# tiddoloos/Scaling-RGCN-training

Hardware: AMD Instinct MI355X
Metric: edges/s per RGCN layer (fwd+bwd) (higher is better)
Workload: dtype f32 (contraction: bf16x3 split of fp32 operands, fp32 accumulate)

## Files before the change

scaling_rgcn_training_amd/csrc/rgcn_dw_tile.hip:

```cpp
#include "rgcn_kernels_shared.h"

namespace rgcn {

constexpr int kDwTileT = 320;
constexpr int kDwTileWalkers = 64;
constexpr int kDwTileMaxRel = 32;
constexpr int kDwFlushUnits = 128;

struct DwTileArgs {
    const int* rel_order;
    const int* chunk_cnt;
    const int* chunk_tile;
    const int* slot_src;
    const float* slot_w;
    const int* slot_row;
    const int* slot_src2;
    const int* walk_ptr;
    const float* x;
    const float* g;
    unsigned x_bytes, g_bytes;
    float* slabs;
    int ldx, ldg, dout4, n_tiles, n_owned, num_rel, walkers;
};

template <bool SPLIT, bool PAIRS = false>
__global__ void __launch_bounds__(512, 2) rgcn_dw_tile_kernel(const DwTileArgs a) {
    constexpr int T = kDwTileT, NP = 64, HS = 8;
    extern __shared__ __attribute__((aligned(16))) float lds[];
    const int tid = threadIdx.x;
    const int lane = tid & 63;
    const int wave = __builtin_amdgcn_readfirstlane(tid >> 6);
    const int quarter = (blockIdx.x >> 3) & 3, p = (blockIdx.x & 7) | ((blockIdx.x >> 5) << 3);
    const int rel = 8 * quarter + wave;
    const bool have = rel < a.num_rel;
    const int t0 = (int)((long)p * a.n_tiles / a.walkers), t1 = (int)((long)(p + 1) * a.n_tiles / a.walkers);
    if (t1 <= t0) return;
    const int i0 = have ? ldc(a.walk_ptr, (long)rel * (a.walkers + 1) + p) : 0;
    const int nun = have ? ldc(a.walk_ptr, (long)rel * (a.walkers + 1) + p + 1) - i0 : 0;
    const int ml = lane & 15, kq = lane >> 4;
    const __amdgpu_buffer_rsrc_t rx = make_rsrc(a.x, a.x_bytes), rg = make_rsrc(a.g, a.g_bytes);
    const unsigned colb = 16u * (unsigned)ml;
    const unsigned rbx = (unsigned)a.ldx * 4u, rbg = (unsigned)a.ldg * 4u;
    const unsigned gcol = ml < a.dout4 ? colb : 0xFFFFFFF0u;
    const unsigned grow = ml < a.dout4 ? rbg : 0u;
    const int perm = kq * 4;
// ... 5 lines not shown
        for (int jb = 0; jb < 4; ++jb) acc[ia][jb] = (f32x4){0.f, 0.f, 0.f, 0.f};

    auto dma_tile = [&](int t, int b) {
        float* base = lds + b * T * NP;
        for (int i = wave; i < T / 4; i += 8) {
            const unsigned row = (unsigned)(t * T + 4 * i + kq);
            dma16_buf(rg, __umul24(row, grow) + gcol, base + i * 4 * NP);
        }
    };
    struct Idx {
        int h, g;
        float w;
        int h2;
    };
    auto unit_of = [&](int k) { return ldc(a.rel_order, i0 + (k < nun ? k : (nun > 0 ? nun - 1 : 0))); };
    auto load_idx = [&](int unit) {
        const size_t base = (size_t)unit * kChunk + lane;
        int h2 = 0;
        if constexpr (PAIRS) h2 = a.slot_src2[(size_t)unit * 8 + (lane & 7)];
        return Idx{a.slot_src[base], a.slot_row[base], a.slot_w[base], h2};
    };
    auto issue_half = [&](f32x4 (&a4)[HS], f32x4& pair, const Idx& ix, int h) {
        if constexpr (PAIRS) {
            const int i2 = __builtin_amdgcn_ds_bpermute(perm + 16 * h, ix.h2);
            pair = __builtin_bit_cast(f32x4, __builtin_amdgcn_raw_buffer_load_b128(rx, (int)(__umul24((unsigned)i2, rbx) + colb), 0, 0));
        }
        int ih[HS];
#pragma unroll
        for (int s = 0; s < HS; ++s) ih[s] = __builtin_amdgcn_ds_bpermute(perm + 16 * (HS * h + s), ix.h);
#pragma unroll
        for (int s = 0; s < HS; ++s)
            a4[s] = __builtin_bit_cast(f32x4, __builtin_amdgcn_raw_buffer_load_b128(rx, (int)(__umul24((unsigned)ih[s], rbx) + colb), 0, 0));
    };
    auto compute_half = [&](f32x4 (&a4)[HS], const f32x4& pair, const Idx& ix, int h, int ngrp, int nks, const float* gbuf, int tile_row0) {
        if constexpr (PAIRS) a4[0] += pair;
        const unsigned loc = (unsigned)(ix.g - tile_row0);
        const int goff = (int)((loc < (unsigned)T ? loc : (unsigned)(T - 1)) * (unsigned)(NP * 4));
        float wv[HS];
        f32x4 g4[HS];
#pragma unroll
        for (int s = 0; s < HS; ++s) {
            wv[s] = __builtin_bit_cast(float, __builtin_amdgcn_ds_bpermute(perm + 16 * (HS * h + s), __builtin_bit_cast(int, ix.w)));
            const int o = __builtin_amdgcn_ds_bpermute(perm + 16 * (HS * h + s), goff);
            g4[s] = *(const f32x4*)((const char*)gbuf + o + colb);
        }
#pragma unroll
        for (int gi = 0; gi < 2; ++gi) {
            if (2 * h + gi < ngrp) {
#pragma unroll
                for (int t = 0; t < 4; ++t) {
                    const int s = 4 * gi + t;
                    f32x4 bv = g4[s] * wv[s];
                    asm volatile("s_nop 4" : "+v"(bv));
#pragma unroll
                    for (int ia = 0; ia < 4; ++ia)
#pragma unroll
                        for (int jb = 0; jb < 4; ++jb)
                            asm volatile("v_mfma_f32_16x16x4_f32 %0, %1, %2, %0" : "+v"(acc[ia][jb]) : "v"(a4[s][ia]), "v"(bv[jb]));
                }
            }
        }
    };

    auto compute_half3 = [&](f32x4 (&a4)[HS], const f32x4& pair, const Idx& ix, int h, int ngrp, const float* gbuf, int tile_row0) {
        if (2 * h >= ngrp) return;
        if constexpr (PAIRS) a4[0] += pair;
        const unsigned loc = (unsigned)(ix.g - tile_row0);
        const int goff = (int)((loc < (unsigned)T ? loc : (unsigned)(T - 1)) * (unsigned)(NP * 4));
        float wv[HS];
        f32x4 g4[HS];
#pragma unroll
        for (int s = 0; s < HS; ++s) {
            wv[s] = __builtin_bit_cast(float, __builtin_amdgcn_ds_bpermute(perm + 16 * (HS * h + s), __builtin_bit_cast(int, ix.w)));
            const int o = __builtin_amdgcn_ds_bpermute(perm + 16 * (HS * h + s), goff);
            g4[s] = *(const f32x4*)((const char*)gbuf + o + colb);
        }
        u32x4 ap[3][4];
#pragma unroll
        for (int ia = 0; ia < 4; ++ia) {
            float v0[4], v1[4];
            unsigned pc[4];
#pragma unroll
            for (int jp = 0; jp < 4; ++jp) { v0[jp] = a4[2 * jp][ia]; v1[jp] = a4[2 * jp + 1][ia]; }
#pragma unroll
            for (int piece = 0; piece < 3; ++piece) {
#pragma unroll
                for (int jp = 0; jp < 4; ++jp) pc[jp] = cvt_pk_bf16(v0[jp], v1[jp]);
                __builtin_amdgcn_sched_barrier(0);
#pragma unroll
                for (int jp = 0; jp < 4; ++jp) ap[piece][ia][jp] = pc[jp];
                if (piece < 2) {
#pragma unroll
                    for (int jp = 0; jp < 4; ++jp) {
                        v0[jp] -= __uint_as_float(pc[jp] << 16);
                        v1[jp] -= __uint_as_float(pc[jp] & 0xFFFF0000u);
                    }
                    __builtin_amdgcn_sched_barrier(0);
                }
            }
        }
        constexpr int pa[6] = {2, 1, 1, 0, 0, 0}, pb[6] = {0, 1, 0, 2, 1, 0};
        auto cut_b = [&](int jb, u32x4 (&bp)[3]) {
#pragma unroll
            for (int jp = 0; jp < 4; ++jp) {
                unsigned h_, m_, l_;
                split3_pair(g4[2 * jp][jb] * wv[2 * jp], g4[2 * jp + 1][jb] * wv[2 * jp + 1], h_, m_, l_);
                bp[0][jp] = h_; bp[1][jp] = m_; bp[2][jp] = l_;
            }
        };
// ... 38 lines not shown
                    __builtin_amdgcn_sched_group_barrier(0x002, 3, 0);
                }
            }
            __builtin_amdgcn_sched_barrier(0);
        }
        __builtin_amdgcn_s_setprio(0);
    };

    auto pin_loads = [] { asm volatile("" ::: "memory"); };
    float* const slab = a.slabs + ((size_t)p * a.num_rel + (have ? rel : 0)) * (64 * 64);
    auto fold_into_slab = [&](float sgn) {
        if (!have) return;
        if constexpr (!SPLIT) asm volatile("s_nop 15\n\ts_nop 15" ::: "memory");
#pragma unroll
        for (int ia = 0; ia < 4; ++ia)
#pragma unroll
            for (int r = 0; r < 4; ++r) {
                f32x4* q = (f32x4*)(slab + (4 * (4 * kq + r) + ia) * NP + 4 * ml);
                f32x4 v = *q;
#pragma unroll
                for (int jb = 0; jb < 4; ++jb) {
                    v[jb] += sgn * acc[ia][jb][r];
                    acc[ia][jb][r] = 0.f;
                }
                *q = v;
            }
    };
    float sgn = 1.f;
    const int fold_period = min(SPLIT ? kDwFlushUnits : 4 * kDwFlushUnits, max(16, nun >> 3));
    int fold_left = fold_period;
    dma_tile(t0, 0);
    int k = 0;
    int uid_cur = unit_of(0), uid_nxt = unit_of(1), uid_nn = unit_of(2);
    int cnt_cur = ldc(a.chunk_cnt, uid_cur), tile_cur = nun > 0 ? ldc(a.chunk_tile, uid_cur) : t1;
    int cnt_nxt = ldc(a.chunk_cnt, uid_nxt), tile_nxt = nun > 1 ? ldc(a.chunk_tile, uid_nxt) : t1;
    Idx ix_cur = load_idx(uid_cur), ix_nxt = load_idx(uid_nxt);
    f32x4 s0[HS], s1[HS];
    f32x4 p0 = {0.f, 0.f, 0.f, 0.f}, p1 = {0.f, 0.f, 0.f, 0.f};
    if (nun > 0) issue_half(s0, p0, ix_cur, 0);
    constexpr int kInFlight = 11 + (PAIRS ? 2 : 0);
    bool walked = nun > 0;
    for (int t = t0; t < t1; ++t) {
        if (walked) asm volatile("s_waitcnt vmcnt(%0)" ::"n"(kInFlight) : "memory");
        else asm volatile("s_waitcnt vmcnt(0)" ::: "memory");
        wg_barrier();
        const int b = (t - t0) & 1;
        if (t + 1 < t1) dma_tile(t + 1, b ^ 1);
        walked = false;
        const float* gbuf = lds + b * T * NP;
        while (k < nun && tile_cur == t) {
            const int ngrp = (cnt_cur + 15) >> 4, nks = (cnt_cur + 3) >> 2;
            walked = true;
            issue_half(s1, p1, ix_cur, 1);
            pin_loads();
            __builtin_amdgcn_sched_barrier(0);
            if constexpr (SPLIT) ix_cur.w *= sgn;
            if constexpr (SPLIT) compute_half3(s0, p0, ix_cur, 0, ngrp, gbuf, t * T);
            else compute_half(s0, p0, ix_cur, 0, ngrp, nks, gbuf, t * T);
            __builtin_amdgcn_sched_barrier(0);
            const Idx ix_nn = load_idx(uid_nn);
            issue_half(s0, p0, ix_nxt, 0);
            pin_loads();
            __builtin_amdgcn_sched_barrier(0);
            if constexpr (SPLIT) compute_half3(s1, p1, ix_cur, 1, ngrp, gbuf, t * T);
            else compute_half(s1, p1, ix_cur, 1, ngrp, nks, gbuf, t * T);
            __builtin_amdgcn_sched_barrier(0);
            ++k;
            if (--fold_left == 0) {
                fold_left = fold_period;
                fold_into_slab(sgn);
                if (SPLIT) sgn = -sgn;
            }
            ix_cur = ix_nxt;
            ix_nxt = ix_nn;
            uid_cur = uid_nxt;
            uid_nxt = uid_nn;
            uid_nn = unit_of(k + 2);
            cnt_cur = cnt_nxt;
            tile_cur = k < nun ? tile_nxt : t1;
            cnt_nxt = ldc(a.chunk_cnt, uid_nxt);
            tile_nxt = k + 1 < nun ? ldc(a.chunk_tile, uid_nxt) : t1;
        }
    }
    asm volatile("s_waitcnt vmcnt(0)" ::: "memory");
    asm volatile("s_nop 15\n\ts_nop 15" ::: "memory");
    fold_into_slab(sgn);
}

__global__ void rgcn_dw_walk_table_kernel(const int* __restrict__ rel_order, const int* __restrict__ chunk_rel,
                                          const int* __restrict__ chunk_tile, int n_units, int n_tiles, int num_rel, int walkers,
                                          int* __restrict__ walk_ptr) {
    const int i = blockIdx.x * blockDim.x + threadIdx.x;
    if (i >= num_rel * (walkers + 1)) return;
    const int r = i / (walkers + 1), p = i - r * (walkers + 1);
    const long target = (long)r * n_tiles + (long)p * n_tiles / walkers;
    int lo = 0, hi = n_units;
    while (lo < hi) {
        const int mid = (lo + hi) >> 1;
        const int c = rel_order[mid];
        if ((long)chunk_rel[c] * n_tiles + chunk_tile[c] < target) lo = mid + 1; else hi = mid;
    }
    walk_ptr[i] = lo;
}

__global__ void rgcn_dw_tile_reduce_kernel(const float* __restrict__ slabs, int walkers, int num_rel, int din, int dout,
                                           float* __restrict__ d_weight) {
    const int r = blockIdx.x;
    for (int e = blockIdx.y * blockDim.x + threadIdx.x; e < din * dout; e += gridDim.y * blockDim.x) {
        const int kk = e / dout, n = e - kk * dout;
        float sum = 0.f;
        for (int w = 0; w < walkers; ++w) sum += slabs[((size_t)w * num_rel + r) * (64 * 64) + kk * 64 + n];
        d_weight[(size_t)r * din * dout + e] = sum;
    }
}


// ... 11 lines not shown

extern "C" int rgcn_dw_tiles_walk(const rgcn_plan_t* plan, int32_t* walk_ptr, void* stream) {
    int st;
    if ((st = check_device()) != RGCN_OK) return st;
    if ((st = check_plan(plan)) != RGCN_OK) return st;
    if (walk_ptr == nullptr) return RGCN_ERR_NULL;
    if (plan->tile != kDwTileT || plan->chunk != 64 || (plan->layout != 0 && plan->layout != 5) || plan->num_relations > kDwTileMaxRel) return RGCN_ERR_PLAN;
    const int n = plan->num_relations * (kDwTileWalkers + 1);
    hipLaunchKernelGGL(rgcn_dw_walk_table_kernel, dim3((n + 255) / 256), dim3(256), 0, (hipStream_t)stream, plan->rel_order,
                       plan->chunk_rel, plan->chunk_tile, plan->n_units, plan->n_tiles, plan->num_relations, kDwTileWalkers, walk_ptr);
    return (int)hipGetLastError();
}

extern "C" size_t rgcn_bwd_dw_tiles_workspace_bytes(int num_relations) {
    return num_relations > 0 ? sizeof(float) * (size_t)kDwTileWalkers * num_relations * 64 * 64 : 0;
}

extern "C" int rgcn_bwd_dw_tiles(const rgcn_plan_t* plan, const int32_t* walk_ptr, const float* x, int ldx, int din, const float* g,
                                 int ldg, int dout, void* workspace, size_t workspace_bytes, float* d_weight, unsigned flags,
                                 void* stream) {
    int st = check_plan(plan);
    if (st != RGCN_OK) return st;
    if (!walk_ptr || !x || !g || !workspace || !d_weight) return RGCN_ERR_NULL;
    if ((st = check_stride(ldx, din)) != RGCN_OK) return st;
    if ((st = check_stride(ldg, dout)) != RGCN_OK) return st;
    if (padded_width(din) != 64 || padded_width(dout) != 64) return RGCN_ERR_WIDTH;
    if (plan->tile != kDwTileT || plan->chunk != 64 || (plan->layout != 0 && plan->layout != 5) || plan->num_relations > kDwTileMaxRel) return RGCN_ERR_PLAN;
    if (workspace_bytes < rgcn_bwd_dw_tiles_workspace_bytes(plan->num_relations)) return RGCN_ERR_WORKSPACE;
    if ((st = check_device()) != RGCN_OK) return st;
    DwTileArgs a;
    a.rel_order = plan->rel_order;
    a.chunk_cnt = plan->chunk_cnt;
    a.chunk_tile = plan->chunk_tile;
    a.slot_src = plan->slot_src;
    a.slot_w = plan->slot_w;
    a.slot_row = plan->slot_row;
    a.walk_ptr = walk_ptr;
    a.x = x;
    a.g = g;
    a.x_bytes = buffer_bytes(plan->n_nodes, ldx, flags);
    a.g_bytes = buffer_bytes(plan->n_owned, ldg, flags);
    if (a.x_bytes == 0 || a.g_bytes == 0) return RGCN_ERR_ADDRESS;
    a.slabs = (float*)workspace;
    a.ldx = ldx;
    a.ldg = ldg;
    a.dout4 = (dout + 3) / 4;
    a.n_tiles = plan->n_tiles;
    a.n_owned = plan->n_owned;
    a.num_rel = plan->num_relations;
    a.walkers = kDwTileWalkers;
    hipStream_t s = (hipStream_t)stream;
    const size_t lds = sizeof(float) * 2 * kDwTileT * 64;
    const bool split = (flags & RGCN_FLAG_SPLIT_PRODUCERS) != 0;
    a.slot_src2 = plan->layout == 5 ? plan->slot_src2 : nullptr;
    if (plan->layout == 5 && a.slot_src2 == nullptr) return RGCN_ERR_NULL;
    hipError_t e = split ? allow_full_lds<rgcn_dw_tile_kernel<true>>() : allow_full_lds<rgcn_dw_tile_kernel<false>>();
    if (e != hipSuccess) return (int)e;
    e = hipMemsetAsync(workspace, 0, rgcn_bwd_dw_tiles_workspace_bytes(plan->num_relations), s);
    if (e != hipSuccess) return (int)e;
    if (a.slot_src2 != nullptr) {
        e = split ? allow_full_lds<rgcn_dw_tile_kernel<true, true>>() : allow_full_lds<rgcn_dw_tile_kernel<false, true>>();
        if (e != hipSuccess) return (int)e;
        if (split) hipLaunchKernelGGL((rgcn_dw_tile_kernel<true, true>), dim3(4 * kDwTileWalkers), dim3(512), lds, s, a);
        else hipLaunchKernelGGL((rgcn_dw_tile_kernel<false, true>), dim3(4 * kDwTileWalkers), dim3(512), lds, s, a);
    } else if (split) hipLaunchKernelGGL(rgcn_dw_tile_kernel<true>, dim3(4 * kDwTileWalkers), dim3(512), lds, s, a);
    else hipLaunchKernelGGL(rgcn_dw_tile_kernel<false>, dim3(4 * kDwTileWalkers), dim3(512), lds, s, a);
// ... 5 lines not shown
```

scaling_rgcn_training_amd/csrc/rgcn_plan.hip:

```cpp
#include <hip/hip_runtime.h>
#include <stdint.h>
#include <string.h>
#include "../../include/rgcn_mi355x.h"

namespace rgcn_planner {

typedef unsigned long long u64;
typedef unsigned int u32;

constexpr int kSortItems = 32;
constexpr int kSegKeys = 64 * kSortItems;
constexpr int kSortThreads = 256;
constexpr int kScanThreads = 256;
constexpr int kScanItems = 8;
constexpr int kScanBlock = kScanThreads * kScanItems;

__host__ __device__ inline int bits_for(u64 max_value) {
    int b = 1;
    while ((max_value >> b) != 0 && b < 64) ++b;
    return b;
}

__device__ inline u32 block_exclusive_scan(u32 v, u32* lds_wave_tot, u32& block_total) {
    const int lane = threadIdx.x & 63, wave = threadIdx.x >> 6;
// ... 582 lines not shown
        while (j + len < n && lrow[j + len] == lrow[j] && lw[j + len] == lw[j]) ++len;
        u32 k = 0;
        while (k < len) {
            const bool as_pair = k + 1 < len && pair_left > 0;
            u32 u, sl;
            if (as_pair) {
                u = next_pair[0] < pairs_in[0] ? 0u : 1u;
                const u32 kk = next_pair[u]++;
                sl = kk < 4u ? kk : 28u + kk;
                --pair_left;
            } else {
                u = single_u;
                for (;;) {
                    while (next_single[u] < unit_heads(u) && is_pair_place(u, next_single[u])) ++next_single[u];
                    if (next_single[u] < unit_heads(u)) break;
                    single_u = ++u;
                }
                sl = next_single[u]++;
            }
            const size_t g = base + (size_t)u * 64u + sl;
            slot_src[g] = lsrc[j + k];
            slot_w[g] = __uint_as_float(lw[j + k]);
            slot_row[g] = lrow[j + k];
            if (as_pair) {
                slot_src2[(size_t)(c + u) * 8u + (sl < 4u ? sl : sl - 28u)] = lsrc[j + k + 1];
                k += 2;
            } else {
                k += 1;
            }
        }
        j += len;
    }
    for (u32 i = 0; i < m; ++i) chunk_cnt[c + i] = i < U ? (int32_t)(((unit_heads(i) + 15u) / 16u) * 16u) : 0;
}

__global__ void fill_i32_kernel(int32_t* __restrict__ p, u64 n, int32_t v) {
    const u64 i = (u64)blockIdx.x * blockDim.x + threadIdx.x;
    if (i < n) p[i] = v;
}

__global__ void tile_ptr_kernel(const int32_t* __restrict__ chunk_tile, u32 n_chunks, u32 n_tiles, int32_t* __restrict__ tile_ptr) {
    const u32 t = blockIdx.x * blockDim.x + threadIdx.x;
    if (t > n_tiles) return;
    u32 lo = 0, hi = n_chunks;
    while (lo < hi) {
        const u32 mid = (lo + hi) >> 1;
        if ((u32)chunk_tile[mid] < t) lo = mid + 1; else hi = mid;
    }
    tile_ptr[t] = (int32_t)lo;
}

__global__ void chunk_keys_kernel(const int32_t* __restrict__ chunk_rel, u32 n_chunks, u64* __restrict__ keys, u32* __restrict__ vals) {
    const u32 c = blockIdx.x * blockDim.x + threadIdx.x;
    if (c >= n_chunks) return;
    keys[c] = (u64)(u32)chunk_rel[c];
    vals[c] = c;
}
__global__ void unit_counts_kernel(const u32* __restrict__ order, const int32_t* __restrict__ chunk_cnt, u32 n_chunks, u32* __restrict__ ucnt) {
    const u32 j = blockIdx.x * blockDim.x + threadIdx.x;
    if (j >= n_chunks) return;
    ucnt[j] = ((u32)chunk_cnt[order[j]] + 63u) / 64u;
}
__global__ void emit_units_kernel(const u32* __restrict__ order, const int32_t* __restrict__ chunk_cnt, const u32* __restrict__ uoff,
                                  u32 n_chunks, u32 upc, int32_t* __restrict__ rel_order) {
    const u32 j = blockIdx.x * blockDim.x + threadIdx.x;
    if (j >= n_chunks) return;
// ... 260 lines not shown
    int32_t* chunk_rel = (int32_t*)plan->chunk_rel;
    int32_t* chunk_cnt = (int32_t*)plan->chunk_cnt;
    int32_t* chunk_tile = (int32_t*)plan->chunk_tile;
    int32_t* chunk_flags = (int32_t*)plan->chunk_flags;
    u32* dstl = (u32*)slot_row;
    hipLaunchKernelGGL(fill_slots_kernel, dim3(grid_for(n_slots)), dim3(256), 0, s, n_slots, bs.n_nodes, bs.tile, slot_src, slot_w, dstl);
    u32* split = ws.scan_a;
    const u32 placement = (bs.layout == 2 || bs.layout == 3 || bs.layout == 5) ? 0u : bs.layout;
    hipLaunchKernelGGL(chunk_meta_kernel, dim3(grid_for(bs.n_chunks)), dim3(256), 0, s, ws.gch, ws.gstart, ws.gkey, bs.n_groups,
                       bs.n_chunks, bs.chunk, bs.cap, placement, ws.sb.k[bs.ubuf], bs.kl, split, chunk_rel, chunk_cnt, chunk_tile, chunk_flags);
    hipLaunchKernelGGL(place_kernel, dim3(grid_for(bs.n_unique)), dim3(256), 0, s, ws.sb.k[bs.ubuf], ws.sb.v[bs.ubuf], bs.n_unique,
                       ws.scan_b, ws.gstart, ws.gch, bs.chunk, bs.cap, placement, split, bs.kl, slot_src, slot_w, dstl);
    hipLaunchKernelGGL(row_tile_kernel, dim3(grid_for(n_rt)), dim3(256), 0, s, dstl, n_rt, bs.chunk, bs.tile, bs.n_own, chunk_tile,
                       slot_acc, slot_row, chunk_flags);
    const u32 struct_tile = bs.layout == 2 ? (bs.tile < 32768u ? bs.tile : 32768u) : bs.tile;
    const u32 n_tiles = (bs.n_own + struct_tile - 1) / struct_tile;
    hipLaunchKernelGGL(tile_ptr_kernel, dim3(grid_for((u64)n_tiles + 1)), dim3(256), 0, s, chunk_tile, bs.n_chunks, n_tiles,
                       (int32_t*)plan->tile_ptr);
    if (bs.layout == 5) {
        if (!plan->slot_src2) return RGCN_ERR_NULL;
        hipLaunchKernelGGL(fill_i32_kernel, dim3(grid_for((u64)bs.n_chunks * 8u)), dim3(256), 0, s, (int32_t*)plan->slot_src2, (u64)bs.n_chunks * 8u,
                           (int32_t)bs.n_nodes);
        hipLaunchKernelGGL(dw_pairs_kernel, dim3(grid_for(bs.n_chunks, kPairThreads)), dim3(kPairThreads), 0, s, bs.n_chunks, bs.n_nodes, bs.n_own,
                           chunk_rel, chunk_tile, chunk_cnt, slot_src, slot_w, slot_row, (int32_t*)plan->slot_src2);
    }
    SortBufs cb = ws.sb;
    hipLaunchKernelGGL(chunk_keys_kernel, dim3(grid_for(bs.n_chunks)), dim3(256), 0, s, chunk_rel, bs.n_chunks, cb.k[0], cb.v[0]);
    const int cur = radix_sort_pairs(cb, bs.n_chunks, bs.kl.rel_bits, s);
    u32* ucnt = ws.scan_b;
    hipLaunchKernelGGL(unit_counts_kernel, dim3(grid_for(bs.n_chunks)), dim3(256), 0, s, cb.v[cur], chunk_cnt, bs.n_chunks, ucnt);
    exclusive_scan(ucnt, ucnt, bs.n_chunks, ws.sb.sums, s);
    hipLaunchKernelGGL(emit_units_kernel, dim3(grid_for(bs.n_chunks)), dim3(256), 0, s, cb.v[cur], chunk_cnt, ucnt, bs.n_chunks,
                       bs.chunk / 64u, (int32_t*)plan->rel_order);
    if (bs.layout == 3)
        hipLaunchKernelGGL(compact_runs_kernel, dim3(grid_for(bs.n_chunks, kCompactThreads)), dim3(kCompactThreads), 0, s, bs.n_chunks, bs.n_nodes, bs.tile, bs.n_own,
                           chunk_rel, chunk_tile, chunk_cnt, chunk_flags, slot_src, slot_w, slot_row, slot_acc);
    plan->n_nodes = (int32_t)bs.n_nodes;
    plan->n_owned = (int32_t)bs.n_own;
    plan->num_relations = (int32_t)bs.num_rel;
    plan->tile = (int32_t)struct_tile;
    plan->n_tiles = (int32_t)n_tiles;
    plan->n_chunks = (int32_t)bs.n_chunks;
    plan->chunk = (int32_t)bs.chunk;
    plan->n_units = (int32_t)bs.n_units;
    if (bs.layout == 5) {
        u32 nu = 0;
        const int st = read_u32(ws.sb.sums + scan_blocks(bs.n_chunks), &nu, s);
        if (st != 0) return st;
        plan->n_units = (int32_t)nu;
    }
    plan->layout = (int32_t)bs.layout;
    plan->chunk_rows = (int32_t)(bs.cap * 16u);
    return (int)hipGetLastError();
}

__global__ void slot_keys_kernel(const int32_t* __restrict__ slot_row, u32 n_slots, u64* __restrict__ keys, u32* __restrict__ vals) {
    const u32 i = blockIdx.x * blockDim.x + threadIdx.x;
    if (i >= n_slots) return;
    keys[i] = (u64)(u32)slot_row[i];
    vals[i] = i;
}
__global__ void seg_ptr_kernel(const u64* __restrict__ keys, u32 n_slots, u32 n_owned, int32_t* __restrict__ seg_ptr) {
    const u32 d = blockIdx.x * blockDim.x + threadIdx.x;
    if (d > n_owned) return;
    u32 lo = 0, hi = n_slots;
    while (lo < hi) {
// ... 25 lines not shown
```

scaling_rgcn_training_amd/plan.py:

```python
from __future__ import annotations

import functools
import os as _os

import numpy as np
from dataclasses import dataclass, field
from typing import Dict, Optional, Tuple

import torch
from torch import Tensor

CHUNK = 64
UNIT = 64
CHUNKS = (64, 128)
CHUNK_112 = 112


@dataclass
class TilePlan:
    n_nodes: int
    node_begin: int
    node_end: int
    num_relations: int
    tile: int
# ... 34 lines not shown
            self.tile_ptr, self.chunk_rel, self.chunk_cnt, self.chunk_tile, self.chunk_flags, self.rel_order,
            self.slot_src, self.slot_w, self.slot_row, self.slot_acc))


def edge_weights(src: Tensor, dst: Tensor, rel: Tensor, num_relations: int, aggr: str = "mean") -> Tensor:
    if aggr in ("sum", "add", "max"):
        return torch.ones(dst.shape[0], dtype=torch.float32, device=dst.device)
    if aggr != "mean":
        raise ValueError(f"unsupported aggr {aggr!r}")
    key = dst.to(torch.int64) * num_relations + rel.to(torch.int64)
    skey, perm = torch.sort(key)
    _, inv, cnt = torch.unique_consecutive(skey, return_inverse=True, return_counts=True)
    w_sorted = 1.0 / cnt.to(torch.float32)[inv]
    w = torch.empty_like(w_sorted)
    w[perm] = w_sorted
    return w


def build_plan(gather: Tensor, scatter: Tensor, rel: Tensor, w: Tensor, n_nodes: int,
               num_relations: int, tile: int, node_begin: int = 0,
               node_end: Optional[int] = None, chunk: int = CHUNK, split: bool = False) -> TilePlan:
    cap = None
    if chunk == CHUNK_112:
        if int(split) not in (0, 3):
            raise ValueError("112-row chunks: layouts 0 and 3 only")
        if int(split) == 3:
            return compact_runs(build_plan(gather, scatter, rel, w, n_nodes, num_relations, tile, node_begin, node_end, chunk, False))
        chunk, cap = 128, 7
    if chunk not in CHUNKS:
        raise ValueError(f"chunk must be one of {CHUNKS} (or {CHUNK_112})")
    if int(split) == 5:
        if chunk != 64:
            raise ValueError("layout 5 (pairs on one slot: the tile-major weight-gradient plan) needs 64-slot chunks")
        return dw_pairs(build_plan(gather, scatter, rel, w, n_nodes, num_relations, tile, node_begin, node_end, chunk, False))
    if split and chunk != 128:
        raise ValueError("the team placement and the run compaction need 128-slot chunks")
    if int(split) == 3:
        return compact_runs(build_plan(gather, scatter, rel, w, n_nodes, num_relations, tile, node_begin, node_end, chunk, False))
    CHUNK = chunk
    if node_end is None:
        node_end = n_nodes
    if node_end <= node_begin:
        return empty_plan(n_nodes, node_begin, num_relations, tile, chunk, gather.device, 1 if split else 0)
    if node_begin % tile != 0:
        raise ValueError("node_begin must be a multiple of the tile size")
    dev = gather.device
    n_own = node_end - node_begin
    r1 = num_relations + 1
    gather = gather.to(torch.int64)
    scatter = scatter.to(torch.int64)
    rel = rel.to(torch.int64)
    if rel.numel() and (int(rel.min()) < 0 or int(rel.max()) >= num_relations):
        raise ValueError("edge_type out of range [0, num_relations)")
    if gather.numel() and (int(gather.min()) < 0 or int(gather.max()) >= n_nodes
                           or int(scatter.min()) < 0 or int(scatter.max()) >= n_nodes):
        raise ValueError("edge_index out of range [0, num_nodes)")
    own = (scatter >= node_begin) & (scatter < node_end)
    if not bool(own.all()):
        gather, scatter, rel, w = gather[own], scatter[own], rel[own], w[own]
    n_edges = int(gather.shape[0])
    nodes = torch.arange(node_begin, node_end, device=dev, dtype=torch.int64)
    g_all = torch.cat([gather, nodes])
    loc = torch.cat([scatter, nodes]) - node_begin
    r_all = torch.cat([rel, torch.full((n_own,), num_relations, device=dev, dtype=torch.int64)])
    w_all = torch.cat([w.to(torch.float32), torch.ones(n_own, device=dev, dtype=torch.float32)])
    tile_id = loc // tile
    dstl = loc - tile_id * tile
# ... 251 lines not shown
                    while True:
                        while next_single[u] < unit_heads(u) and is_pair_place(u, next_single[u]):
                            next_single[u] += 1
                        if next_single[u] < unit_heads(u):
                            break
                        u += 1
                        single_u = u
                    sl = next_single[u]
                    next_single[u] += 1
                g = base + u * 64 + sl
                src[g], row[g], wbits[g] = rows[j0 + k]
                if as_pair:
                    src2[(c0 + u) * 8 + (sl if sl < 4 else sl - 28)] = rows[j0 + k + 1][0]
                    k += 2
                else:
                    k += 1
        for i in range(m):
            cnt[c0 + i] = (unit_heads(i) + 15) // 16 * 16 if i < units else 0
    plan.slot_src = torch.from_numpy(src).to(dev)
    plan.slot_w = torch.from_numpy(wbits.view("float32")).to(dev)
    plan.slot_row = torch.from_numpy(row).to(dev)
    plan.chunk_cnt = torch.from_numpy(cnt).to(dev)
    plan.slot_src2 = torch.from_numpy(src2).to(dev)
    if plan.slot_dstl is not None:
        plan.slot_dstl = None
    order_key = plan.chunk_rel.to(torch.int64) * max(plan.n_tiles, 1) + plan.chunk_tile.to(torch.int64)
    chunk_order = torch.sort(order_key, stable=True)[1]
    used = plan.chunk_cnt.to(torch.int64)[chunk_order] > 0
    plan.rel_order = chunk_order[used].to(torch.int32)
    plan.layout = 5
    return plan


def team_placement(dstl: Tensor, gcnt: Tensor, grp_of_edge: Tensor, rank: Tensor, chunk_base: Tensor,
                   grp_of_chunk: Tensor, idx_in_grp: Tensor):
    C, g16 = 128, ROWS_PER_MFMA_TILE
    dev = dstl.device
    n_chunks = int(grp_of_chunk.shape[0])
    n_c = torch.clamp(gcnt[grp_of_chunk] - idx_in_grp * C, max=C)
    nt = (n_c + (g16 - 1)) // g16
    n_a = (nt + 1) // 2
    n_b = nt - n_a
    two = nt > 1
    lo_c = torch.clamp(n_c - g16 * n_b, min=1)
    hi_c = torch.minimum(n_c - 1, g16 * n_a)
    mid_c = (lo_c + hi_c + 1) // 2
    cidx = rank // C
    jc = rank - cidx * C
    chunk_of_row = chunk_base[grp_of_edge] + cidx
    prev_dstl = torch.cat([dstl[:1], dstl[:-1]])
    boundary = (jc >= 1) & (dstl != prev_dstl)
    cand = boundary & two[chunk_of_row] & (jc >= lo_c[chunk_of_row]) & (jc <= hi_c[chunk_of_row])
    dist = jc - mid_c[chunk_of_row]
    score = 2 * dist.abs() + (dist > 0).to(torch.int64)
    big_score = 1 << 20
    best = torch.full((n_chunks,), big_score, dtype=torch.int64, device=dev)
    best = best.scatter_reduce(0, chunk_of_row[cand], score[cand], reduce="amin", include_self=True)
    has = best < big_score
    k = best // 2
    s_found = torch.where(best % 2 == 1, mid_c + k, mid_c - k)
    s_c = torch.where(two, torch.where(has, s_found, mid_c), n_c)
    straddle = two & ~has
    chunk_cnt = (nt * g16).to(torch.int32)
    s_r = s_c[chunk_of_row]
    na_r, nb_r = n_a[chunk_of_row], torch.clamp(n_b[chunk_of_row], min=1)
    j1 = torch.clamp(jc - s_r, min=0)
# ... 299 lines not shown
```

Baseline: 4.398 billion.

## Pack weight-gradient units across adjacent tiles to cut padded slots

Adds a packing pass, on both the GPU plan builder and the Python plan, that repacks layout-5 units so each unit may hold edges from two consecutive destination tiles. Per-unit flags record which halves straddle a tile boundary. The dW tile kernel is restructured to step tiles inside the unit walk and merge gradient rows from the next tile's LDS buffer, with vmcnt waits tracked by a count of outstanding loads. The aim is fewer partly filled, padded units and so fewer wasted MFMA and gather operations, at the cost of more complex control flow, extra mid-unit barriers and a heavier plan build.

Result: faster. 4.494 billion, median of 6 (+2.2%).

```diff
diff --git a/scaling_rgcn_training_amd/csrc/rgcn_dw_tile.hip b/scaling_rgcn_training_amd/csrc/rgcn_dw_tile.hip
--- a/scaling_rgcn_training_amd/csrc/rgcn_dw_tile.hip
+++ b/scaling_rgcn_training_amd/csrc/rgcn_dw_tile.hip
@@ -11,6 +11,7 @@
     const int* rel_order;
     const int* chunk_cnt;
     const int* chunk_tile;
+    const int* chunk_flags;
     const int* slot_src;
     const float* slot_w;
     const int* slot_row;
@@ -82,18 +83,27 @@
         for (int s = 0; s < HS; ++s)
             a4[s] = __builtin_bit_cast(f32x4, __builtin_amdgcn_raw_buffer_load_b128(rx, (int)(__umul24((unsigned)ih[s], rbx) + colb), 0, 0));
     };
-    auto compute_half = [&](f32x4 (&a4)[HS], const f32x4& pair, const Idx& ix, int h, int ngrp, int nks, const float* gbuf, int tile_row0) {
-        if constexpr (PAIRS) a4[0] += pair;
+    auto gather_g = [&](f32x4 (&g4)[HS], float (&wv)[HS], const Idx& ix, int h, const float* gbuf, int tile_row0) {
         const unsigned loc = (unsigned)(ix.g - tile_row0);
         const int goff = (int)((loc < (unsigned)T ? loc : (unsigned)(T - 1)) * (unsigned)(NP * 4));
-        float wv[HS];
-        f32x4 g4[HS];
 #pragma unroll
         for (int s = 0; s < HS; ++s) {
             wv[s] = __builtin_bit_cast(float, __builtin_amdgcn_ds_bpermute(perm + 16 * (HS * h + s), __builtin_bit_cast(int, ix.w)));
             const int o = __builtin_amdgcn_ds_bpermute(perm + 16 * (HS * h + s), goff);
             g4[s] = *(const f32x4*)((const char*)gbuf + o + colb);
         }
+    };
+    auto merge_g = [&](f32x4 (&g4)[HS], const Idx& ix, int h, const float* gbuf, int tile_row0) {
+        const unsigned loc = (unsigned)(ix.g - tile_row0);
+        const int goff = loc < (unsigned)T ? (int)(loc * (unsigned)(NP * 4)) : -1;
+#pragma unroll
+        for (int s = 0; s < HS; ++s) {
+            const int o = __builtin_amdgcn_ds_bpermute(perm + 16 * (HS * h + s), goff);
+            if (o >= 0) g4[s] = *(const f32x4*)((const char*)gbuf + o + colb);
+        }
+    };
+    auto compute_half = [&](f32x4 (&a4)[HS], const f32x4& pair, const f32x4 (&g4)[HS], const float (&wv)[HS], int h, int ngrp, int nks) {
+        if constexpr (PAIRS) a4[0] += pair;
 #pragma unroll
         for (int gi = 0; gi < 2; ++gi) {
             if (2 * h + gi < ngrp) {
@@ -112,19 +122,8 @@
         }
     };
 
-    auto compute_half3 = [&](f32x4 (&a4)[HS], const f32x4& pair, const Idx& ix, int h, int ngrp, const float* gbuf, int tile_row0) {
-        if (2 * h >= ngrp) return;
+    auto compute_half3 = [&](f32x4 (&a4)[HS], const f32x4& pair, const f32x4 (&g4)[HS], const float (&wv)[HS]) {
         if constexpr (PAIRS) a4[0] += pair;
-        const unsigned loc = (unsigned)(ix.g - tile_row0);
-        const int goff = (int)((loc < (unsigned)T ? loc : (unsigned)(T - 1)) * (unsigned)(NP * 4));
-        float wv[HS];
-        f32x4 g4[HS];
-#pragma unroll
-        for (int s = 0; s < HS; ++s) {
-            wv[s] = __builtin_bit_cast(float, __builtin_amdgcn_ds_bpermute(perm + 16 * (HS * h + s), __builtin_bit_cast(int, ix.w)));
-            const int o = __builtin_amdgcn_ds_bpermute(perm + 16 * (HS * h + s), goff);
-            g4[s] = *(const f32x4*)((const char*)gbuf + o + colb);
-        }
         u32x4 ap[3][4];
 #pragma unroll
         for (int ia = 0; ia < 4; ++ia) {
@@ -229,56 +228,88 @@
     dma_tile(t0, 0);
     int k = 0;
     int uid_cur = unit_of(0), uid_nxt = unit_of(1), uid_nn = unit_of(2);
-    int cnt_cur = ldc(a.chunk_cnt, uid_cur), tile_cur = nun > 0 ? ldc(a.chunk_tile, uid_cur) : t1;
-    int cnt_nxt = ldc(a.chunk_cnt, uid_nxt), tile_nxt = nun > 1 ? ldc(a.chunk_tile, uid_nxt) : t1;
+    int cnt_cur = ldc(a.chunk_cnt, uid_cur), tile_cur = nun > 0 ? ldc(a.chunk_tile, uid_cur) : t1, flg_cur = ldc(a.chunk_flags, uid_cur);
+    int cnt_nxt = ldc(a.chunk_cnt, uid_nxt), tile_nxt = nun > 1 ? ldc(a.chunk_tile, uid_nxt) : t1, flg_nxt = ldc(a.chunk_flags, uid_nxt);
     Idx ix_cur = load_idx(uid_cur), ix_nxt = load_idx(uid_nxt);
     f32x4 s0[HS], s1[HS];
     f32x4 p0 = {0.f, 0.f, 0.f, 0.f}, p1 = {0.f, 0.f, 0.f, 0.f};
     if (nun > 0) issue_half(s0, p0, ix_cur, 0);
-    constexpr int kInFlight = 11 + (PAIRS ? 2 : 0);
-    bool walked = nun > 0;
-    for (int t = t0; t < t1; ++t) {
-        if (walked) asm volatile("s_waitcnt vmcnt(%0)" ::"n"(kInFlight) : "memory");
+    constexpr int kHalfOps = 8 + (PAIRS ? 1 : 0), kIdxOps = 3 + (PAIRS ? 1 : 0);
+    constexpr int kInFlight = kHalfOps + kIdxOps;
+    int since = nun > 0 ? kHalfOps + 2 * kIdxOps : 0;
+    int t = t0 - 1;
+    const float* gbuf = lds;
+    auto step_tile = [&] {
+        if (t + 1 >= t1) return;
+        ++t;
+        if (since >= kInFlight + kHalfOps) asm volatile("s_waitcnt vmcnt(%0)" ::"n"(kInFlight + kHalfOps) : "memory");
+        else if (since >= kInFlight) asm volatile("s_waitcnt vmcnt(%0)" ::"n"(kInFlight) : "memory");
+        else if (since >= kHalfOps) asm volatile("s_waitcnt vmcnt(%0)" ::"n"(kHalfOps) : "memory");
         else asm volatile("s_waitcnt vmcnt(0)" ::: "memory");
         wg_barrier();
         const int b = (t - t0) & 1;
         if (t + 1 < t1) dma_tile(t + 1, b ^ 1);
-        walked = false;
-        const float* gbuf = lds + b * T * NP;
-        while (k < nun && tile_cur == t) {
-            const int ngrp = (cnt_cur + 15) >> 4, nks = (cnt_cur + 3) >> 2;
-            walked = true;
-            issue_half(s1, p1, ix_cur, 1);
-            pin_loads();
-            __builtin_amdgcn_sched_barrier(0);
-            if constexpr (SPLIT) ix_cur.w *= sgn;
-            if constexpr (SPLIT) compute_half3(s0, p0, ix_cur, 0, ngrp, gbuf, t * T);
-            else compute_half(s0, p0, ix_cur, 0, ngrp, nks, gbuf, t * T);
-            __builtin_amdgcn_sched_barrier(0);
-            const Idx ix_nn = load_idx(uid_nn);
-            issue_half(s0, p0, ix_nxt, 0);
-            pin_loads();
-            __builtin_amdgcn_sched_barrier(0);
-            if constexpr (SPLIT) compute_half3(s1, p1, ix_cur, 1, ngrp, gbuf, t * T);
-            else compute_half(s1, p1, ix_cur, 1, ngrp, nks, gbuf, t * T);
-            __builtin_amdgcn_sched_barrier(0);
-            ++k;
-            if (--fold_left == 0) {
-                fold_left = fold_period;
-                fold_into_slab(sgn);
-                if (SPLIT) sgn = -sgn;
-            }
-            ix_cur = ix_nxt;
-            ix_nxt = ix_nn;
-            uid_cur = uid_nxt;
-            uid_nxt = uid_nn;
-            uid_nn = unit_of(k + 2);
-            cnt_cur = cnt_nxt;
-            tile_cur = k < nun ? tile_nxt : t1;
-            cnt_nxt = ldc(a.chunk_cnt, uid_nxt);
-            tile_nxt = k + 1 < nun ? ldc(a.chunk_tile, uid_nxt) : t1;
-        }
+        since = 0;
+        gbuf = lds + b * T * NP;
+    };
+    constexpr int kH0Straddles = 1 << 28, kH1Straddles = 1 << 29, kH1Next = 1 << 30;
+    while (k < nun) {
+        while (t < tile_cur && t + 1 < t1) step_tile();
+        const int ngrp = (cnt_cur + 15) >> 4, nks = (cnt_cur + 3) >> 2;
+        issue_half(s1, p1, ix_cur, 1);
+        since += kHalfOps;
+        pin_loads();
+        __builtin_amdgcn_sched_barrier(0);
+        if constexpr (SPLIT) ix_cur.w *= sgn;
+        if (!SPLIT || 0 < ngrp) {
+            float wv[HS];
+            f32x4 g4[HS];
+            gather_g(g4, wv, ix_cur, 0, gbuf, t * T);
+            if (flg_cur & kH0Straddles) {
+                step_tile();
+                merge_g(g4, ix_cur, 0, gbuf, t * T);
+            }
+            if constexpr (SPLIT) compute_half3(s0, p0, g4, wv);
+            else compute_half(s0, p0, g4, wv, 0, ngrp, nks);
+        }
+        __builtin_amdgcn_sched_barrier(0);
+        const Idx ix_nn = load_idx(uid_nn);
+        issue_half(s0, p0, ix_nxt, 0);
+        since += kHalfOps + kIdxOps;
+        pin_loads();
+        __builtin_amdgcn_sched_barrier(0);
+        if (!SPLIT || 2 < ngrp) {
+            float wv[HS];
+            f32x4 g4[HS];
+            if (flg_cur & kH1Next) step_tile();
+            gather_g(g4, wv, ix_cur, 1, gbuf, t * T);
+            if (flg_cur & kH1Straddles) {
+                step_tile();
+                merge_g(g4, ix_cur, 1, gbuf, t * T);
+            }
+            if constexpr (SPLIT) compute_half3(s1, p1, g4, wv);
+            else compute_half(s1, p1, g4, wv, 1, ngrp, nks);
+        }
+        __builtin_amdgcn_sched_barrier(0);
+        ++k;
+        if (--fold_left == 0) {
+            fold_left = fold_period;
+            fold_into_slab(sgn);
+            if (SPLIT) sgn = -sgn;
+        }
+        ix_cur = ix_nxt;
+        ix_nxt = ix_nn;
+        uid_cur = uid_nxt;
+        uid_nxt = uid_nn;
+        uid_nn = unit_of(k + 2);
+        cnt_cur = cnt_nxt;
+        flg_cur = flg_nxt;
+        tile_cur = k < nun ? tile_nxt : t1;
+        cnt_nxt = ldc(a.chunk_cnt, uid_nxt);
+        flg_nxt = ldc(a.chunk_flags, uid_nxt);
+        tile_nxt = k + 1 < nun ? ldc(a.chunk_tile, uid_nxt) : t1;
     }
+    while (t + 1 < t1) step_tile();
     asm volatile("s_waitcnt vmcnt(0)" ::: "memory");
     asm volatile("s_nop 15\n\ts_nop 15" ::: "memory");
     fold_into_slab(sgn);
@@ -356,6 +387,7 @@
     a.rel_order = plan->rel_order;
     a.chunk_cnt = plan->chunk_cnt;
     a.chunk_tile = plan->chunk_tile;
+    a.chunk_flags = plan->chunk_flags;
     a.slot_src = plan->slot_src;
     a.slot_w = plan->slot_w;
     a.slot_row = plan->slot_row;
diff --git a/scaling_rgcn_training_amd/csrc/rgcn_plan.hip b/scaling_rgcn_training_amd/csrc/rgcn_plan.hip
--- a/scaling_rgcn_training_amd/csrc/rgcn_plan.hip
+++ b/scaling_rgcn_training_amd/csrc/rgcn_plan.hip
@@ -638,6 +638,161 @@
         j += len;
     }
     for (u32 i = 0; i < m; ++i) chunk_cnt[c + i] = i < U ? (int32_t)(((unit_heads(i) + 15u) / 16u) * 16u) : 0;
+}
+
+constexpr u32 kDwWalkers = 64;
+constexpr int32_t kDwFlagH0Straddles = 1 << 28;
+constexpr int32_t kDwFlagH1Straddles = 1 << 29;
+constexpr int32_t kDwFlagH1Next = 1 << 30;
+__global__ void __launch_bounds__(64) dw_pack_kernel(const u32* __restrict__ n_units_ptr, u32 n_tiles, u32 walkers, u32 n_nodes, u32 n_own,
+                                                     const int32_t* __restrict__ rel_order, const int32_t* __restrict__ chunk_rel,
+                                                     int32_t* chunk_tile, int32_t* __restrict__ chunk_cnt, int32_t* __restrict__ chunk_flags,
+                                                     int32_t* __restrict__ slot_src, float* __restrict__ slot_w, int32_t* __restrict__ slot_row,
+                                                     int32_t* __restrict__ slot_src2) {
+    const u32 r = blockIdx.x / walkers, p = blockIdx.x % walkers;
+    const u32 t0 = (u32)((u64)p * n_tiles / walkers), t1 = (u32)((u64)(p + 1) * n_tiles / walkers);
+    if (t1 - t0 < 2u) return;
+    const u32 n_units = *n_units_ptr;
+    auto lower = [&](u32 tile) {
+        const u64 target = (u64)r * n_tiles + tile;
+        u32 lo = 0, hi = n_units;
+        while (lo < hi) {
+            const u32 mid = (lo + hi) >> 1;
+            const int32_t c = rel_order[mid];
+            if ((u64)(u32)chunk_rel[c] * n_tiles + (u32)((volatile int32_t*)chunk_tile)[c] < target) lo = mid + 1; else hi = mid;
+        }
+        return lo;
+    };
+    const u32 i0 = lower(t0), n = lower(t1) - i0;
+    if (n < 2u) return;
+    __shared__ int32_t i_src[64], i_row[64], i_s2[8], q_src[32], q_row[32], p_src[4], p_row[4], p_s2[4];
+    __shared__ u32 i_w[64], q_w[32], p_w[4], s_j, s_bad;
+    const u32 lane = threadIdx.x;
+    u32 j = 0, hh = 0, np = 0, ns = 0, cur_i = 0, n_half[2] = {0u, 0u}, tmask = 0;
+    bool open = false, bad = false;
+    int32_t ut = 0;
+    auto pad_half = [&](u32 u, u32 h, u32 from) {
+        for (u32 q = from; q < 32u; ++q) {
+            const size_t g = (size_t)u * 64u + 32u * h + q;
+            slot_src[g] = (int32_t)n_nodes;
+            slot_w[g] = 0.f;
+            slot_row[g] = (int32_t)n_own;
+        }
+    };
+    auto close_unit = [&]() {
+        const u32 u = (u32)rel_order[i0 + j];
+        if (hh == 1u) {
+            pad_half(u, 1u, 0u);
+            for (u32 q = 0; q < 4u; ++q) slot_src2[(size_t)u * 8u + 4u + q] = (int32_t)n_nodes;
+        }
+        const u32 used = n_half[1] ? 32u + n_half[1] : n_half[0];
+        chunk_cnt[u] = (int32_t)(((used + 15u) / 16u) * 16u);
+        chunk_tile[u] = ut;
+        const bool a0 = tmask & 1u, b0 = tmask & 2u, a1 = tmask & 4u, b1 = tmask & 8u;
+        chunk_flags[u] = (a0 && b0 ? kDwFlagH0Straddles : 0) | (a1 && b1 ? kDwFlagH1Straddles : 0) | (b1 && !a1 && !b0 ? kDwFlagH1Next : 0);
+        ++j;
+        open = false;
+    };
+    auto close_half = [&]() {
+        const u32 u = (u32)rel_order[i0 + j];
+        const size_t base = (size_t)u * 64u + 32u * hh;
+        for (u32 q = 0; q < 4u; ++q) {
+            if (q < np) {
+                slot_src[base + q] = p_src[q];
+                slot_w[base + q] = __uint_as_float(p_w[q]);
+                slot_row[base + q] = p_row[q];
+            }
+            slot_src2[(size_t)u * 8u + 4u * hh + q] = q < np ? p_s2[q] : (int32_t)n_nodes;
+        }
+        for (u32 q = 0; q < ns; ++q) {
+            slot_src[base + np + q] = q_src[q];
+            slot_w[base + np + q] = __uint_as_float(q_w[q]);
+            slot_row[base + np + q] = q_row[q];
+        }
+        pad_half(u, hh, np + ns);
+        n_half[hh] = np + ns;
+        np = ns = 0;
+        if (++hh == 2u) close_unit();
+    };
+    auto enter = [&](int32_t th) {
+        if (open && th > ut + 1) {
+            if (np + ns > 0u) close_half();
+            if (open) close_unit();
+        }
+        if (!open) {
+            if (j > cur_i) { bad = true; return; }
+            open = true;
+            ut = th;
+            hh = 0;
+            n_half[0] = n_half[1] = 0;
+            tmask = 0;
+        }
+        tmask |= 1u << (2u * hh + (u32)(th - ut));
+    };
+    auto put_single = [&](int32_t s, int32_t rw, u32 w, int32_t th) {
+        enter(th);
+        if (bad) return;
+        q_src[ns] = s;
+        q_row[ns] = rw;
+        q_w[ns] = w;
+        ++ns;
+        if (np + ns == 32u) close_half();
+    };
+    for (u32 i = 0; i < n; ++i) {
+        const u32 u = (u32)rel_order[i0 + i];
+        const int32_t ti = chunk_tile[u];
+        i_src[lane] = slot_src[(size_t)u * 64u + lane];
+        i_row[lane] = slot_row[(size_t)u * 64u + lane];
+        i_w[lane] = __float_as_uint(slot_w[(size_t)u * 64u + lane]);
+        if (lane < 8u) i_s2[lane] = slot_src2[(size_t)u * 8u + lane];
+        __syncthreads();
+        if (lane == 0u) {
+            cur_i = i;
+            for (u32 s = 0; s < 64u && !bad; ++s) {
+                const int32_t sv = i_src[s];
+                if ((u32)sv == n_nodes) continue;
+                const int32_t rw = i_row[s];
+                const u32 w = i_w[s];
+                const int32_t s2 = s < 4u ? i_s2[s] : (s >= 32u && s < 36u ? i_s2[s - 28u] : (int32_t)n_nodes);
+                if ((u32)s2 == n_nodes) {
+                    put_single(sv, rw, w, ti);
+                    continue;
+                }
+                enter(ti);
+                if (bad) break;
+                if (np == 4u) {
+                    put_single(sv, rw, w, ti);
+                    put_single(s2, rw, w, ti);
+                    continue;
+                }
+                p_src[np] = sv;
+                p_row[np] = rw;
+                p_w[np] = w;
+                p_s2[np] = s2;
+                ++np;
+                if (np + ns == 32u) close_half();
+            }
+            if (i + 1u == n && !bad && open) {
+                if (np + ns > 0u) close_half();
+                if (open) close_unit();
+            }
+            s_j = j;
+            s_bad = bad ? 1u : 0u;
+        }
+        __syncthreads();
+        if (s_bad) return;
+    }
+    for (u32 jj = s_j; jj < n; ++jj) {
+        const u32 u = (u32)rel_order[i0 + jj];
+        slot_src[(size_t)u * 64u + lane] = (int32_t)n_nodes;
+        slot_w[(size_t)u * 64u + lane] = 0.f;
+        slot_row[(size_t)u * 64u + lane] = (int32_t)n_own;
+        if (lane < 8u) slot_src2[(size_t)u * 8u + lane] = (int32_t)n_nodes;
+        if (lane == 0u) {
+            chunk_cnt[u] = 0;
+            chunk_flags[u] = 0;
+        }
+    }
 }
 
 __global__ void fill_i32_kernel(int32_t* __restrict__ p, u64 n, int32_t v) {
@@ -964,6 +1119,15 @@
     exclusive_scan(ucnt, ucnt, bs.n_chunks, ws.sb.sums, s);
     hipLaunchKernelGGL(emit_units_kernel, dim3(grid_for(bs.n_chunks)), dim3(256), 0, s, cb.v[cur], chunk_cnt, ucnt, bs.n_chunks,
                        bs.chunk / 64u, (int32_t*)plan->rel_order);
+    if (bs.layout == 5 && bs.num_rel > 0) {
+        hipLaunchKernelGGL(dw_pack_kernel, dim3(bs.num_rel * kDwWalkers), dim3(64), 0, s, ws.sb.sums + scan_blocks(bs.n_chunks), n_tiles,
+                           kDwWalkers, bs.n_nodes, bs.n_own, (const int32_t*)plan->rel_order, chunk_rel, chunk_tile, chunk_cnt, chunk_flags,
+                           slot_src, slot_w, slot_row, (int32_t*)plan->slot_src2);
+        hipLaunchKernelGGL(unit_counts_kernel, dim3(grid_for(bs.n_chunks)), dim3(256), 0, s, cb.v[cur], chunk_cnt, bs.n_chunks, ucnt);
+        exclusive_scan(ucnt, ucnt, bs.n_chunks, ws.sb.sums, s);
+        hipLaunchKernelGGL(emit_units_kernel, dim3(grid_for(bs.n_chunks)), dim3(256), 0, s, cb.v[cur], chunk_cnt, ucnt, bs.n_chunks,
+                           bs.chunk / 64u, (int32_t*)plan->rel_order);
+    }
     if (bs.layout == 3)
         hipLaunchKernelGGL(compact_runs_kernel, dim3(grid_for(bs.n_chunks, kCompactThreads)), dim3(kCompactThreads), 0, s, bs.n_chunks, bs.n_nodes, bs.tile, bs.n_own,
                            chunk_rel, chunk_tile, chunk_cnt, chunk_flags, slot_src, slot_w, slot_row, slot_acc);
diff --git a/scaling_rgcn_training_amd/plan.py b/scaling_rgcn_training_amd/plan.py
--- a/scaling_rgcn_training_amd/plan.py
+++ b/scaling_rgcn_training_amd/plan.py
@@ -90,7 +90,7 @@
     if int(split) == 5:
         if chunk != 64:
             raise ValueError("layout 5 (pairs on one slot: the tile-major weight-gradient plan) needs 64-slot chunks")
-        return dw_pairs(build_plan(gather, scatter, rel, w, n_nodes, num_relations, tile, node_begin, node_end, chunk, False))
+        return dw_pack(dw_pairs(build_plan(gather, scatter, rel, w, n_nodes, num_relations, tile, node_begin, node_end, chunk, False)))
     if split and chunk != 128:
         raise ValueError("the team placement and the run compaction need 128-slot chunks")
     if int(split) == 3:
@@ -408,6 +408,127 @@
     return plan
 
 
+DW_WALKERS = 64
+DW_FLAG_H0_STRADDLES = 1 << 28
+DW_FLAG_H1_STRADDLES = 1 << 29
+DW_FLAG_H1_NEXT = 1 << 30
+
+
+def dw_pack(plan: TilePlan, walkers: int = DW_WALKERS) -> TilePlan:
+    if plan.chunk != 64 or plan.layout != 5:
+        raise ValueError("dw_pack wants a layout-5 plan")
+    dev = plan.slot_src.device
+    n_nodes, n_own, n_tiles = plan.n_nodes, plan.n_owned, plan.n_tiles
+    src = plan.slot_src.cpu().numpy().copy()
+    wbits = plan.slot_w.cpu().numpy().copy().view("uint32")
+    row = plan.slot_row.cpu().numpy().copy()
+    src2 = plan.slot_src2.cpu().numpy().copy()
+    cnt = plan.chunk_cnt.cpu().numpy().copy()
+    ctile = plan.chunk_tile.cpu().numpy().copy()
+    flags = plan.chunk_flags.cpu().numpy().copy()
+    crel = plan.chunk_rel.cpu().numpy()
+    order = plan.rel_order.cpu().numpy().astype(np.int64)
+    key = crel.astype(np.int64)[order] * max(n_tiles, 1) + ctile.astype(np.int64)[order]
+
+    def pack_stream(units):
+        st = {"j": 0, "open": False, "ut": 0, "hh": 0, "n": [0, 0], "t1": [[False, False], [False, False]]}
+        pairs, singles = [], []
+        o_src, o_row, o_w, o_s2 = [None], [None], [None], [None]
+
+        def open_unit(th):
+            st.update(open=True, ut=th, hh=0, n=[0, 0], t1=[[False, False], [False, False]])
+            o_src[0] = np.full(64, n_nodes, np.int32)
+            o_row[0] = np.full(64, n_own, np.int32)
+            o_w[0] = np.zeros(64, np.uint32)
+            o_s2[0] = np.full(8, n_nodes, np.int32)
+
+        def close_half():
+            hh, b = st["hh"], 32 * st["hh"]
+            for q, (s_, r_, w_, s2_) in enumerate(pairs):
+                o_src[0][b + q], o_row[0][b + q], o_w[0][b + q], o_s2[0][4 * hh + q] = s_, r_, w_, s2_
+            for q, (s_, r_, w_) in enumerate(singles):
+                o_src[0][b + len(pairs) + q], o_row[0][b + len(pairs) + q], o_w[0][b + len(pairs) + q] = s_, r_, w_
+            st["n"][hh] = len(pairs) + len(singles)
+            pairs.clear()
+            singles.clear()
+            st["hh"] = hh + 1
+            if hh == 1:
+                close_unit()
+
+        def close_unit():
+            if pairs or singles:
+                close_half()
+                if not st["open"]:
+                    return
+            u = units[st["j"]]
+            assert st["j"] <= st["i"], "dw_pack: output overtook input"
+            n0, n1 = st["n"]
+            src[64 * u:64 * u + 64], row[64 * u:64 * u + 64], wbits[64 * u:64 * u + 64] = o_src[0], o_row[0], o_w[0]
+            src2[8 * u:8 * u + 8] = o_s2[0]
+            cnt[u] = ((32 + n1 if n1 else n0) + 15) // 16 * 16
+            ctile[u] = st["ut"]
+            (a0, b0), (a1, b1) = st["t1"]
+            flags[u] = ((DW_FLAG_H0_STRADDLES if a0 and b0 else 0) | (DW_FLAG_H1_STRADDLES if a1 and b1 else 0)
+                        | (DW_FLAG_H1_NEXT if b1 and not a1 and not b0 else 0))
+            st["j"] += 1
+            st["open"] = False
+
+        def put(s_, r_, w_, s2_, th):
+            if st["open"] and th > st["ut"] + 1:
+                close_unit()
+            if not st["open"]:
+                open_unit(th)
+            if s2_ is not None and len(pairs) == 4:
+                put(s_, r_, w_, None, th)
+                put(s2_, r_, w_, None, th)
+                return
+            st["t1"][st["hh"]][th - st["ut"]] = True
+            if s2_ is not None:
+                pairs.append((s_, r_, w_, s2_))
+            else:
+                singles.append((s_, r_, w_))
+            if len(pairs) + len(singles) == 32:
+                close_half()
+
+        for i, u in enumerate(units):
+            st["i"] = i
+            i_src, i_row, i_w = src[64 * u:64 * u + 64].copy(), row[64 * u:64 * u + 64].copy(), wbits[64 * u:64 * u + 64].copy()
+            i_s2, ti = src2[8 * u:8 * u + 8].copy(), int(ctile[u])
+            for s in range(64):
+                if i_src[s] == n_nodes:
+                    continue
+                k = s if s < 4 else (s - 28 if 32 <= s < 36 else -1)
+                put(i_src[s], i_row[s], i_w[s], int(i_s2[k]) if k >= 0 and i_s2[k] != n_nodes else None, ti)
+        st["i"] = len(units)
+        if st["open"]:
+            close_unit()
+        for jj in range(st["j"], len(units)):
+            u = units[jj]
+            src[64 * u:64 * u + 64], row[64 * u:64 * u + 64], wbits[64 * u:64 * u + 64] = n_nodes, n_own, 0
+            src2[8 * u:8 * u + 8] = n_nodes
+            cnt[u], flags[u] = 0, 0
+
+    for r in range(plan.num_relations):
+        for p in range(walkers):
+            t0, t1 = p * n_tiles // walkers, (p + 1) * n_tiles // walkers
+            if t1 - t0 < 2:
+                continue
+            i0, i1 = np.searchsorted(key, [r * n_tiles + t0, r * n_tiles + t1])
+            if i1 - i0 >= 2:
+                pack_stream(order[i0:i1])
+    plan.slot_src = torch.from_numpy(src).to(dev)
+    plan.slot_w = torch.from_numpy(wbits.view("float32")).to(dev)
+    plan.slot_row = torch.from_numpy(row).to(dev)
+    plan.slot_src2 = torch.from_numpy(src2).to(dev)
+    plan.chunk_cnt = torch.from_numpy(cnt).to(dev)
+    plan.chunk_tile = torch.from_numpy(ctile).to(dev)
+    plan.chunk_flags = torch.from_numpy(flags).to(dev)
+    chunk_order = torch.sort(plan.chunk_rel.to(torch.int64), stable=True)[1]
+    used = plan.chunk_cnt.to(torch.int64)[chunk_order] > 0
+    plan.rel_order = chunk_order[used].to(torch.int32)
+    return plan
+
+
 def team_placement(dstl: Tensor, gcnt: Tensor, grp_of_edge: Tensor, rank: Tensor, chunk_base: Tensor,
                    grp_of_chunk: Tensor, idx_in_grp: Tensor):
     C, g16 = 128, ROWS_PER_MFMA_TILE
```
